# facebookresearch/jepa

Measured on AMD Instinct MI355X. Metric: V-JEPA pretrain clips/sec (fwd+bwd+EMA), higher is better.
Workload: dtype bf16; 1 GPU; V-JEPA pretrain step ViT-L/16 16x224x224, B=24/GPU, 2 multiblock masks (vitl16.yaml); global_batch=24, per_gpu_batch=24, parallelism=dp1, hw_queues=4

## Files before the change

### jepa_amd/csrc/attention.hip

```cpp
#include "attn_common.hpp"

template <int HDP, int NBUF, int RS>
__global__ __launch_bounds__(256) void attn_fwd_sm_kernel(const bf16_t* __restrict__ qkv_all,
                                                          bf16_t* __restrict__ o_all, float* __restrict__ lse2_all,
                                                          AttnSegs sg, int H, int hd, float sc) {
  constexpr int QT = 2, NT = 256;
  using RT = RowTile<HDP, NT>;
  constexpr int DIST = NBUF - 1;
  static_assert(RT::CAN_FULL, "tile items must be a multiple of the workgroup size");
  constexpr bool PSUM = RS == 1;
  constexpr int NDMA = RT::NIT, BUFB = 2 * RT::BYTES;
  __shared__ __attribute__((aligned(16))) char smem[NBUF * BUFB];
  const TrFrag<HDP> trf(threadIdx.x & 63);
  constexpr int KS = HDP / 32, DT = HeadTiles<HDP>::DT;
  const int tid = threadIdx.x, lane = tid & 63, w = tid >> 6;
  const int li = lane & 15, g = lane >> 4;
  const AttnWg wg = attn_wg(sg, H);
  const int S = wg.S, qb = wg.blk;
  const int64_t rs = (int64_t)3 * H * hd, os = (int64_t)H * hd;
  const bf16_t* qbase = wg.rows(qkv_all, rs, hd);
  const bf16_t* kbase = qbase + os;
  const int q0 = qb * 128 + w * (16 * QT);

  bf16x8_t qf[QT][KS];
#pragma unroll
  for (int qt = 0; qt < QT; qt++)
#pragma unroll
    for (int ks = 0; ks < KS; ks++) {
      const int q = q0 + qt * 16 + li, d0 = ks * 32 + 8 * g;
      qf[qt][ks] = scale_frag(load_frag_global(qbase + (int64_t)q * rs + d0, q < S && d0 < hd), sc);
    }

  f32x4_t oacc[QT][DT];
#pragma unroll
  for (int qt = 0; qt < QT; qt++)
#pragma unroll
    for (int dt = 0; dt < DT; dt++) oacc[qt][dt] = (f32x4_t){0.f, 0.f, 0.f, 0.f};
  float mrun[QT], lrun[QT];
  f32x4_t lacc[QT];
  f32x4_t seed[QT];
#pragma unroll
  for (int qt = 0; qt < QT; qt++) {
    mrun[qt] = 0.f;
    lrun[qt] = 0.f;
    lacc[qt] = (f32x4_t){0.f, 0.f, 0.f, 0.f};
    seed[qt] = (f32x4_t){0.f, 0.f, 0.f, 0.f};
  }

  const int nt = (S + 63) / 64;
  const TileDma<HDP, NT, PSUM> dma(tid, hd);
  if constexpr (PSUM) dma.template fill_ypad<NBUF>(smem, tid);
  auto issue = [&](const int tile, const int buf_off, auto full_tag) {
    const bf16_t* kt = kbase + (int64_t)tile * 64 * rs;
    dma.template issue<decltype(full_tag)::value>(kt, rs, kt + os, rs, 0, S - tile * 64, smem + buf_off);
  };
  __builtin_amdgcn_s_waitcnt(0x0f70);
#pragma unroll
  for (int d = 0; d < DIST; d++)
    if (d < nt) issue(d, d * BUFB, std::false_type{});
  RingCursor<NBUF, BUFB> ring;
  const bool wave_live = qb * 128 + dma.wu * (16 * QT) < S;

  auto iter = [&](const int t, auto fast_tag, auto first_tag) {
    constexpr bool FAST = decltype(fast_tag)::value, FIRST = decltype(first_tag)::value;
    const int k0 = t * 64;
    char* k_lds = smem + ring.cur;
    char* v_lds = k_lds + RT::BYTES;
    if (DIST >= 2 && (FAST || t + 1 < nt)) wait_vmcnt<2 * NDMA>();
    else wait_vmcnt<0>();
    lgkm_barrier();
    if constexpr (FAST) issue(t + DIST, ring.nxt, std::true_type{});
    else if (t + DIST < nt) issue(t + DIST, ring.nxt, std::false_type{});
    ring.advance();
    if (!wave_live) return;
    f32x4_t sacc[QT][4];
#pragma unroll
    for (int kt = 0; kt < 4; kt++)
#pragma unroll
      for (int ks = 0; ks < KS; ks++) {
        const bf16x8_t kf = RT::frag(k_lds, kt * 16 + li, ks * 4 + g);
#pragma unroll
        for (int qt = 0; qt < QT; qt++)
          sacc[qt][kt] = __builtin_amdgcn_mfma_f32_16x16x32_bf16(kf, qf[qt][ks], ks == 0 ? seed[qt] : sacc[qt][kt], 0, 0, 0);
      }
    if constexpr (!FAST) {
      if (k0 + 64 > S) {
#pragma unroll
        for (int qt = 0; qt < QT; qt++)
#pragma unroll
          for (int kt = 0; kt < 4; kt++)
#pragma unroll
            for (int r = 0; r < 4; r++)
              if (k0 + kt * 16 + 4 * g + r >= S) sacc[qt][kt][r] = -INFINITY;
      }
    }
    u32x4_t pw[QT][2];
    f32x2_t ls2[QT];
    auto exps = [&](const int qt) __attribute__((always_inline)) {
      ls2[qt] = (f32x2_t){0.f, 0.f};
#pragma unroll
      for (int c = 0; c < 2; c++)
#pragma unroll
        for (int k2 = 0; k2 < 2; k2++)
#pragma unroll
          for (int hf = 0; hf < 2; hf++) {
            const int kt = 2 * c + k2;
            const f32x2_t e = {__builtin_amdgcn_exp2f(sacc[qt][kt][2 * hf]), __builtin_amdgcn_exp2f(sacc[qt][kt][2 * hf + 1])};
            if constexpr (RS == 0) ls2[qt] += e;
            pw[qt][c][2 * k2 + hf] = cvt_pk_bf16(e[0], e[1]);
          }
    };
    bool rebase = FIRST;
    if constexpr (!FIRST) {
      uint32_t orw = 0;
#pragma unroll
      for (int qt = 0; qt < QT; qt++) {
        exps(qt);
        orw |= (pw[qt][0][0] | pw[qt][0][1] | pw[qt][0][2]) | (pw[qt][0][3] | pw[qt][1][0] | pw[qt][1][1]) |
               (pw[qt][1][2] | pw[qt][1][3]);
      }
      rebase = __any((orw & 0x40004000u) != 0);
    }
    if (rebase) {
#pragma unroll
      for (int qt = 0; qt < QT; qt++) {
        float mx = -INFINITY;
#pragma unroll
        for (int kt = 0; kt < 4; kt++)
#pragma unroll
          for (int r = 0; r < 4; r++) mx = fmaxf(mx, sacc[qt][kt][r]);
        mx = fmaxf(mx, __shfl_xor(mx, 16, 64));
        mx = fmaxf(mx, __shfl_xor(mx, 32, 64));
        float shift = mx + SM_HEADROOM;
        if constexpr (!FIRST) {
          shift = fmaxf(shift, 0.f);
          const float alpha = __builtin_amdgcn_exp2f(-shift);
          lrun[qt] *= alpha;
          if constexpr (RS == 2) lacc[qt] *= alpha;
#pragma unroll
          for (int dt = 0; dt < DT; dt++) oacc[qt][dt] *= alpha;
        }
        mrun[qt] += shift;
        seed[qt] = (f32x4_t){-mrun[qt], -mrun[qt], -mrun[qt], -mrun[qt]};
#pragma unroll
        for (int kt = 0; kt < 4; kt++) sacc[qt][kt] -= (f32x4_t){shift, shift, shift, shift};
        exps(qt);
      }
    }
    bf16x8_t pf[QT][2];
#pragma unroll
    for (int qt = 0; qt < QT; qt++) {
      if constexpr (RS == 0) lrun[qt] += ls2[qt][0] + ls2[qt][1];
      pf[qt][0] = __builtin_bit_cast(bf16x8_t, pw[qt][0]);
      pf[qt][1] = __builtin_bit_cast(bf16x8_t, pw[qt][1]);
    }
#pragma unroll
    for (int c = 0; c < 2; c++)
#pragma unroll
      for (int dt = 0; dt < DT; dt++) {
        const bf16x8_t vf = trf.load(v_lds, c * 32, dt * 16);
#pragma unroll
        for (int qt = 0; qt < QT; qt++)
          oacc[qt][dt] = __builtin_amdgcn_mfma_f32_16x16x32_bf16(vf, pf[qt][c], oacc[qt][dt], 0, 0, 0);
      }
    if constexpr (RS == 2) {
      const u32x4_t one4 = {0x3F803F80u, 0x3F803F80u, 0x3F803F80u, 0x3F803F80u};
      const bf16x8_t ones = __builtin_bit_cast(bf16x8_t, one4);
#pragma unroll
      for (int c = 0; c < 2; c++)
#pragma unroll
        for (int qt = 0; qt < QT; qt++) lacc[qt] = __builtin_amdgcn_mfma_f32_16x16x32_bf16(ones, pf[qt][c], lacc[qt], 0, 0, 0);
    }
  };
  const int nfull = S / 64;
  const int t_fast = nfull - DIST > 0 ? nfull - DIST : 0;
  int t = 1;
  if (t_fast > 0) iter(0, std::true_type{}, std::true_type{});
  else iter(0, std::false_type{}, std::true_type{});
  for (; t < t_fast; t++) iter(t, std::true_type{}, std::false_type{});
  for (; t < nt; t++) iter(t, std::false_type{}, std::false_type{});

#pragma unroll
  for (int qt = 0; qt < QT; qt++) {
    float l;
    if constexpr (PSUM) {
      l = __shfl(oacc[qt][1][0], 32 + li, 64);
    } else if constexpr (RS == 2) {
      l = lacc[qt][0];
    } else {
      l = lrun[qt];
      l += __shfl_xor(l, 16, 64);
      l += __shfl_xor(l, 32, 64);
    }
    const int q = q0 + qt * 16 + li;
    if (q < S) {
      store_acc_row<DT>(wg.rows(o_all, os, hd) + q * os, oacc[qt], g, hd, 1.0f / l);
      if (g == 0 && lse2_all) wg.stats(lse2_all, H)[q] = mrun[qt] + log2f(l);
    }
  }
}

template <int HDP, int KT>
__global__ __launch_bounds__(256) void attn_bwd_dkdv_kernel(const bf16_t* __restrict__ qkv_all,
                                                            const bf16_t* __restrict__ dout_all,
                                                            const float* __restrict__ lse2_all,
                                                            const float* __restrict__ delta_all,
                                                            bf16_t* __restrict__ dqkv_all, AttnSegs sg, int H, int hd,
                                                            float sc, float scale, float* __restrict__ colkv) {
  constexpr int BUFB = 2 * RowTile<HDP>::BYTES;
  __shared__ __attribute__((aligned(16))) char smem[2 * BUFB + 2 * 2 * 64 * 4];
  float* stat = (float*)(smem + 2 * BUFB);
  const TrFrag<HDP> trf(threadIdx.x & 63);
  constexpr int KS = HDP / 32, DT = HeadTiles<HDP>::DT;
  const int tid = threadIdx.x, lane = tid & 63, w = tid >> 6;
  const int li = lane & 15, g = lane >> 4;
  const AttnWg wg = attn_wg(sg, H);
  const int S = wg.S, kb = wg.blk;
  const int64_t rs = (int64_t)3 * H * hd, os = (int64_t)H * hd;
  const bf16_t* qbase = wg.rows(qkv_all, rs, hd);
  const bf16_t* kbase = qbase + os;
  const bf16_t* vbase = kbase + os;
  const bf16_t* dobase = wg.rows(dout_all, os, hd);
  const float* lse_b = wg.stats(lse2_all, H);
  const float* dl_b = wg.stats(delta_all, H);
  int key[KT];
  bool key_ok[KT];
#pragma unroll
  for (int kt = 0; kt < KT; kt++) {
    key[kt] = kb * (64 * KT) + (w * KT + kt) * 16 + li;
    key_ok[kt] = key[kt] < S;
  }

  bf16x8_t kf[KT][KS], vf[KT][KS];
#pragma unroll
  for (int kt = 0; kt < KT; kt++)
#pragma unroll
    for (int ks = 0; ks < KS; ks++) {
      const int d0 = ks * 32 + 8 * g;
      kf[kt][ks] = load_frag_global(kbase + (int64_t)key[kt] * rs + d0, key_ok[kt] && d0 < hd);
      vf[kt][ks] = load_frag_global(vbase + (int64_t)key[kt] * rs + d0, key_ok[kt] && d0 < hd);
      kf[kt][ks] = scale_frag(kf[kt][ks], sc);
    }
  f32x4_t dvacc[KT][DT], dkacc[KT][DT];
#pragma unroll
  for (int kt = 0; kt < KT; kt++)
#pragma unroll
    for (int dt = 0; dt < DT; dt++) {
      dvacc[kt][dt] = (f32x4_t){0.f, 0.f, 0.f, 0.f};
      dkacc[kt][dt] = (f32x4_t){0.f, 0.f, 0.f, 0.f};
    }

  float lse_r = 0.f, dl_r = 0.f;
  const int nt = (S + 63) / 64;
  const bool wave_live = kb * (64 * KT) + __builtin_amdgcn_readfirstlane(w) * (16 * KT) < S;
  const TileDma<HDP, 256> dma(tid, hd);
  auto load_stats = [&](int r0) {
    if (tid < 64) {
      const int q = r0 + tid;
      lse_r = q < S ? lse_b[q] : INFINITY;
      dl_r = q < S ? -dl_b[q] : 0.f;
    }
  };
  __builtin_amdgcn_s_waitcnt(0x0f70);
  load_stats(0);
  dma.template issue<false>(qbase, rs, dobase, os, 0, S, smem);
  if (tid < 64) {
    stat[tid] = lse_r;
    stat[64 + tid] = dl_r;
  }
  if (nt > 1) load_stats(64);

  for (int t = 0; t < nt; t++) {
    char* q_lds = smem + (t & 1) * BUFB;
    char* do_lds = q_lds + RowTile<HDP>::BYTES;
    const float* lse_s = stat + (t & 1) * 128;
    const float* dl_s = lse_s + 64;
    wait_vmcnt<0>();
    lgkm_barrier();
    if (t + 1 < nt) {
      if (tid < 64) {
        stat[((t + 1) & 1) * 128 + tid] = lse_r;
        stat[((t + 1) & 1) * 128 + 64 + tid] = dl_r;
      }
      if (t + 2 < nt) load_stats((t + 2) * 64);
      if ((t + 1) * 64 + 64 <= S) dma.template issue<true>(qbase, rs, dobase, os, (t + 1) * 64, S, smem + ((t + 1) & 1) * BUFB);
      else dma.template issue<false>(qbase, rs, dobase, os, (t + 1) * 64, S, smem + ((t + 1) & 1) * BUFB);
    }

    if (!wave_live) continue;
#pragma unroll
    for (int c = 0; c < 2; c++) {
      if (c == 1 && t * 64 + 32 >= S) break;
      float pv[KT][2][4], dsv[KT][2][4];
#pragma unroll
      for (int q2 = 0; q2 < 2; q2++) {
        const int qt = 2 * c + q2;
        const float4 lse4 = *(const float4*)(lse_s + qt * 16 + 4 * g);
        const float4 ndl4 = *(const float4*)(dl_s + qt * 16 + 4 * g);
        f32x4_t sacc[KT], dpacc[KT];
#pragma unroll
        for (int kt = 0; kt < KT; kt++) {
          sacc[kt] = (f32x4_t){-lse4.x, -lse4.y, -lse4.z, -lse4.w};
          dpacc[kt] = (f32x4_t){ndl4.x, ndl4.y, ndl4.z, ndl4.w};
        }
#pragma unroll
        for (int ks = 0; ks < KS; ks++) {
          const bf16x8_t qa = RowTile<HDP>::frag(q_lds, qt * 16 + li, ks * 4 + g);
          const bf16x8_t da = RowTile<HDP>::frag(do_lds, qt * 16 + li, ks * 4 + g);
#pragma unroll
          for (int kt = 0; kt < KT; kt++) {
            sacc[kt] = __builtin_amdgcn_mfma_f32_16x16x32_bf16(qa, kf[kt][ks], sacc[kt], 0, 0, 0);
            dpacc[kt] = __builtin_amdgcn_mfma_f32_16x16x32_bf16(da, vf[kt][ks], dpacc[kt], 0, 0, 0);
          }
        }
#pragma unroll
        for (int kt = 0; kt < KT; kt++)
#pragma unroll
          for (int hf = 0; hf < 2; hf++) {
            const f32x2_t dpv = {dpacc[kt][2 * hf], dpacc[kt][2 * hf + 1]};
            const f32x2_t e = {__builtin_amdgcn_exp2f(sacc[kt][2 * hf]), __builtin_amdgcn_exp2f(sacc[kt][2 * hf + 1])};
            const f32x2_t ds = e * dpv;
            pv[kt][q2][2 * hf] = e[0];
            pv[kt][q2][2 * hf + 1] = e[1];
            dsv[kt][q2][2 * hf] = ds[0];
            dsv[kt][q2][2 * hf + 1] = ds[1];
          }
      }
      bf16x8_t pfr[KT], dfr[KT];
#pragma unroll
      for (int kt = 0; kt < KT; kt++) {
        pfr[kt] = pack_frag(pv[kt][0], pv[kt][1]);
        dfr[kt] = pack_frag(dsv[kt][0], dsv[kt][1]);
      }
#pragma unroll
      for (int dt = 0; dt < DT; dt++) {
        const bf16x8_t dot_f = trf.load(do_lds, c * 32, dt * 16);
        const bf16x8_t qt_f = trf.load(q_lds, c * 32, dt * 16);
#pragma unroll
        for (int kt = 0; kt < KT; kt++) {
          dvacc[kt][dt] = __builtin_amdgcn_mfma_f32_16x16x32_bf16(dot_f, pfr[kt], dvacc[kt][dt], 0, 0, 0);
          dkacc[kt][dt] = __builtin_amdgcn_mfma_f32_16x16x32_bf16(qt_f, dfr[kt], dkacc[kt][dt], 0, 0, 0);
        }
      }
    }
  }

  if (colkv != nullptr) {
    float ck[DT][4], cv[DT][4];
#pragma unroll
    for (int dt = 0; dt < DT; dt++)
#pragma unroll
      for (int r = 0; r < 4; r++) {
        float a = 0.f, c = 0.f;
#pragma unroll
        for (int kt = 0; kt < KT; kt++) {
          a += key_ok[kt] ? dkacc[kt][dt][r] : 0.f;
          c += key_ok[kt] ? dvacc[kt][dt][r] : 0.f;
        }
        ck[dt][r] = row16_sum(a);
        cv[dt][r] = row16_sum(c);
      }
    lgkm_barrier();
    float* red = (float*)smem;
    if (li == 0) {
#pragma unroll
      for (int dt = 0; dt < DT; dt++)
#pragma unroll
        for (int r = 0; r < 4; r++) {
          red[(w * 2 + 0) * HDP + dt * 16 + 4 * g + r] = ck[dt][r];
          red[(w * 2 + 1) * HDP + dt * 16 + 4 * g + r] = cv[dt][r];
        }
    }
    lgkm_barrier();
    if (tid < 2 * HDP) {
      const int which = tid / HDP, d = tid % HDP;
      if (d < hd) {
        float t = red[(0 * 2 + which) * HDP + d] + red[(1 * 2 + which) * HDP + d] + red[(2 * 2 + which) * HDP + d] +
                  red[(3 * 2 + which) * HDP + d];
        if (which == 0) t *= scale;
        wg.colrow(colkv, 2 * os, hd)[(int64_t)which * os + d] = t;
      }
    }
  }
#pragma unroll
  for (int kt = 0; kt < KT; kt++) {
    if (key_ok[kt]) {
      bf16_t* dkp = wg.rows(dqkv_all, rs, hd) + key[kt] * rs + os;
      bf16_t* dvp = dkp + os;
#pragma unroll
      for (int dt = 0; dt < DT; dt++) {
        const int d = dt * 16 + 4 * g;
        if (d < hd) {
          u32x2_t a, c;
          a[0] = cvt_pk_bf16(dkacc[kt][dt][0] * scale, dkacc[kt][dt][1] * scale);
          a[1] = cvt_pk_bf16(dkacc[kt][dt][2] * scale, dkacc[kt][dt][3] * scale);
          c[0] = cvt_pk_bf16(dvacc[kt][dt][0], dvacc[kt][dt][1]);
          c[1] = cvt_pk_bf16(dvacc[kt][dt][2], dvacc[kt][dt][3]);
          *(u32x2_t*)(dkp + d) = a;
          *(u32x2_t*)(dvp + d) = c;
        }
      }
    }
  }
}

template <int HDP>
__global__ __launch_bounds__(256) void attn_bwd_dq_kernel(const bf16_t* __restrict__ qkv_all,
                                                          const bf16_t* __restrict__ o_all,
                                                          const bf16_t* __restrict__ dout_all,
                                                          const float* __restrict__ lse2_all,
                                                          float* __restrict__ delta_all,
                                                          bf16_t* __restrict__ dqkv_all, AttnSegs sg, int H, int hd,
                                                          float sc, float scale, float* __restrict__ colq) {
  constexpr int NBUF = HDP <= 64 ? 3 : 2, DIST = NBUF - 1, BUFB = 2 * RowTile<HDP>::BYTES;
  __shared__ __attribute__((aligned(16))) char smem[NBUF * BUFB];
  const TrFrag<HDP> trf(threadIdx.x & 63);
  constexpr int KS = HDP / 32, DT = HeadTiles<HDP>::DT;
  constexpr int QW = 2;
  const int tid = threadIdx.x, lane = tid & 63, w = tid >> 6;
  const int li = lane & 15, g = lane >> 4;
  const AttnWg wg = attn_wg(sg, H);
  const int S = wg.S, qb = wg.blk;
  const int64_t rs = (int64_t)3 * H * hd, os = (int64_t)H * hd;
  const bf16_t* qbase = wg.rows(qkv_all, rs, hd);
  const bf16_t* kbase = qbase + os;
  const bf16_t* vbase = kbase + os;
  const bf16_t* dobase = wg.rows(dout_all, os, hd);
  const bf16_t* obase = wg.rows(o_all, os, hd);
  const float* lse_b = wg.stats(lse2_all, H);
  float* dl_b = wg.stats(delta_all, H);
  const int q0 = qb * (64 * QW) + w * (16 * QW);

  bf16x8_t qf[QW][KS], dof[QW][KS];
  float lse_q[QW], dl_q[QW];
#pragma unroll
  for (int qt = 0; qt < QW; qt++) {
    const int q = q0 + qt * 16 + li;
    float dsum = 0.f;
#pragma unroll
    for (int ks = 0; ks < KS; ks++) {
      const int d0 = ks * 32 + 8 * g;
      const bool ok = q < S && d0 < hd;
      qf[qt][ks] = load_frag_global(qbase + (int64_t)q * rs + d0, ok);
      dof[qt][ks] = load_frag_global(dobase + (int64_t)q * os + d0, ok);
      const u32x4_t ov = __builtin_bit_cast(u32x4_t, load_frag_global(obase + (int64_t)q * os + d0, ok));
      const u32x4_t dv = __builtin_bit_cast(u32x4_t, dof[qt][ks]);
#pragma unroll
      for (int j = 0; j < 4; j++) dsum += bf_lo(ov[j]) * bf_lo(dv[j]) + bf_hi(ov[j]) * bf_hi(dv[j]);
    }
    dsum += __shfl_xor(dsum, 16, 64);
    dsum += __shfl_xor(dsum, 32, 64);
    lse_q[qt] = q < S ? lse_b[q] : INFINITY;
    dl_q[qt] = q < S ? dsum : 0.f;
    if (g == 0 && q < S) dl_b[q] = dsum;
#pragma unroll
    for (int ks = 0; ks < KS; ks++) qf[qt][ks] = scale_frag(qf[qt][ks], sc);
  }
  f32x4_t dqacc[QW][DT];
#pragma unroll
  for (int qt = 0; qt < QW; qt++)
#pragma unroll
    for (int dt = 0; dt < DT; dt++) dqacc[qt][dt] = (f32x4_t){0.f, 0.f, 0.f, 0.f};

  f32x4_t ndl4[QW];
  f32x4_t nls4[QW];
#pragma unroll
  for (int qt = 0; qt < QW; qt++) {
    ndl4[qt] = (f32x4_t){-dl_q[qt], -dl_q[qt], -dl_q[qt], -dl_q[qt]};
    nls4[qt] = (f32x4_t){-lse_q[qt], -lse_q[qt], -lse_q[qt], -lse_q[qt]};
  }
  const int nt = (S + 63) / 64;
  const bool wave_live = qb * (64 * QW) + __builtin_amdgcn_readfirstlane(w) * (16 * QW) < S;
  const TileDma<HDP, 256> dma(tid, hd);
  constexpr int NDMA2 = 2 * TileDma<HDP, 256>::NDMA;
  __builtin_amdgcn_s_waitcnt(0x0f70);
#pragma unroll
  for (int d = 0; d < DIST; d++)
    if (d < nt) dma.template issue<false>(kbase, rs, vbase, rs, d * 64, S, smem + d * BUFB);
  RingCursor<NBUF, BUFB> ring;

  for (int t = 0; t < nt; t++) {
    const int k0 = t * 64;
    char* k_lds = smem + ring.cur;
    char* v_lds = k_lds + RowTile<HDP>::BYTES;
    if (DIST >= 2 && t + 1 < nt) wait_vmcnt<NDMA2>();
    else wait_vmcnt<0>();
    lgkm_barrier();
    if (t + DIST < nt) {
      if ((t + DIST) * 64 + 64 <= S) dma.template issue<true>(kbase, rs, vbase, rs, (t + DIST) * 64, S, smem + ring.nxt);
      else dma.template issue<false>(kbase, rs, vbase, rs, (t + DIST) * 64, S, smem + ring.nxt);
    }
    ring.advance();
    if (!wave_live) continue;
#pragma unroll
    for (int c = 0; c < 2; c++) {
      if (c == 1 && k0 + 32 >= S) break;
      f32x4_t sacc[QW][2], dpacc[QW][2];
#pragma unroll
      for (int qt = 0; qt < QW; qt++)
#pragma unroll
        for (int k2 = 0; k2 < 2; k2++) {
          sacc[qt][k2] = nls4[qt];
          dpacc[qt][k2] = ndl4[qt];
        }
#pragma unroll
      for (int k2 = 0; k2 < 2; k2++)
#pragma unroll
        for (int ks = 0; ks < KS; ks++) {
          const int kt = 2 * c + k2;
          const bf16x8_t ka = RowTile<HDP>::frag(k_lds, kt * 16 + li, ks * 4 + g);
          const bf16x8_t va = RowTile<HDP>::frag(v_lds, kt * 16 + li, ks * 4 + g);
#pragma unroll
          for (int qt = 0; qt < QW; qt++) {
            sacc[qt][k2] = __builtin_amdgcn_mfma_f32_16x16x32_bf16(ka, qf[qt][ks], sacc[qt][k2], 0, 0, 0);
            dpacc[qt][k2] = __builtin_amdgcn_mfma_f32_16x16x32_bf16(va, dof[qt][ks], dpacc[qt][k2], 0, 0, 0);
          }
        }
#pragma unroll
      for (int qt = 0; qt < QW; qt++) {
#pragma unroll
        for (int k2 = 0; k2 < 2; k2++)
#pragma unroll
          for (int hf = 0; hf < 2; hf++) {
            const f32x2_t sv = {sacc[qt][k2][2 * hf], sacc[qt][k2][2 * hf + 1]};
            const f32x2_t dpv = {dpacc[qt][k2][2 * hf], dpacc[qt][k2][2 * hf + 1]};
            const f32x2_t e = {__builtin_amdgcn_exp2f(sv[0]), __builtin_amdgcn_exp2f(sv[1])};
            const f32x2_t ds = e * dpv;
            sacc[qt][k2][2 * hf] = ds[0];
            sacc[qt][k2][2 * hf + 1] = ds[1];
          }
      }
      if (k0 + 64 > S) {
        asm volatile("" ::: "memory");
#pragma unroll
        for (int qt = 0; qt < QW; qt++)
#pragma unroll
          for (int k2 = 0; k2 < 2; k2++)
#pragma unroll
            for (int r = 0; r < 4; r++)
              if (k0 + (2 * c + k2) * 16 + 4 * g + r >= S) sacc[qt][k2][r] = 0.f;
      }
      bf16x8_t dsf[QW];
#pragma unroll
      for (int qt = 0; qt < QW; qt++) dsf[qt] = pack_frag(sacc[qt][0], sacc[qt][1]);
#pragma unroll
      for (int dt = 0; dt < DT; dt++) {
        const bf16x8_t ktf = trf.load(k_lds, c * 32, dt * 16);
#pragma unroll
        for (int qt = 0; qt < QW; qt++)
          dqacc[qt][dt] = __builtin_amdgcn_mfma_f32_16x16x32_bf16(ktf, dsf[qt], dqacc[qt][dt], 0, 0, 0);
      }
    }
  }

  if (colq != nullptr) {
    float cq[DT][4];
#pragma unroll
    for (int dt = 0; dt < DT; dt++)
#pragma unroll
      for (int r = 0; r < 4; r++) {
        cq[dt][r] = row16_sum(dqacc[0][dt][r] + dqacc[1][dt][r]);
      }
    lgkm_barrier();
    float* red = (float*)smem;
    if (li == 0) {
#pragma unroll
      for (int dt = 0; dt < DT; dt++)
#pragma unroll
        for (int r = 0; r < 4; r++) red[w * HDP + dt * 16 + 4 * g + r] = cq[dt][r];
    }
    lgkm_barrier();
    if (tid < hd) wg.colrow(colq, os, hd)[tid] =
        (red[tid] + red[HDP + tid] + red[2 * HDP + tid] + red[3 * HDP + tid]) * scale;
  }
#pragma unroll
  for (int qt = 0; qt < QW; qt++) {
    const int q = q0 + qt * 16 + li;
    if (q < S) store_acc_row<DT>(wg.rows(dqkv_all, rs, hd) + q * rs, dqacc[qt], g, hd, scale);
  }
}

static int pick_hdp(int64_t hd) { return hd <= 32 ? 32 : (hd <= 64 ? 64 : (hd <= 80 ? 96 : (hd <= 128 ? 128 : 0))); }
constexpr float LOG2E = 1.4426950408889634f;
static int attn_check_hd(const char* who, int64_t hd) {
  VJ_CHECK_ARG(hd % 8 == 0 && pick_hdp(hd) != 0, "%s: head_dim=%ld unsupported (need %%8==0, <=128)", who, (long)hd);
  return 0;
}

template <int HDP_, int NBUF_, int RS_, int KT_>
struct AttnClass { static constexpr int HDP = HDP_, NBUF = NBUF_, RS = RS_, KT = KT_; };
template <class F>
static inline int with_head_dim(int64_t hd, F&& f) {
  switch (pick_hdp(hd)) {
    case 32: return hd == 24 ? f(AttnClass<32, 3, 1, 2>{}) : f(AttnClass<32, 3, 2, 2>{});
    case 64: return f(AttnClass<64, 2, 2, 1>{});
    case 96: return f(AttnClass<96, 2, 2, 1>{});
    default: return f(AttnClass<128, 2, 2, 1>{});
  }
}
static int dkdv_kt(int64_t hd) { return with_head_dim(hd, [](auto c) { return decltype(c)::KT; }); }
static int64_t attn_rows_end(const vj_seg_t* segs, int64_t n_segs) {
  int64_t rows_end = 0;
  for (int64_t i = 0; i < n_segs; i++)
    if (segs[i].B * segs[i].S > 0 && segs[i].row0 + segs[i].B * segs[i].S > rows_end) rows_end = segs[i].row0 + segs[i].B * segs[i].S;
  return rows_end;
}

static int make_segs(const vj_seg_t* segs, int64_t n_segs, int64_t H, int64_t rows_per_block, AttnSegs* out, int64_t* nblk,
                     const char* who) {
  VJ_CHECK_ARG(segs != nullptr && n_segs >= 1 && n_segs <= VJ_ATTN_MAX_SEGS, "%s: 1..%d segments", who, VJ_ATTN_MAX_SEGS);
  int k = 0;
  int64_t tot = 0, col = 0;
  for (int64_t i = 0; i < n_segs; i++) {
    VJ_CHECK_ARG(segs[i].B >= 0 && segs[i].S >= 0 && segs[i].row0 >= 0, "%s: bad segment %ld", who, (long)i);
    if (segs[i].B * segs[i].S == 0) continue;
    const int64_t nb = cdiv64(segs[i].S, rows_per_block);
    tot += segs[i].B * H * nb;
    VJ_CHECK_ARG(tot < (1ll << 31) && segs[i].S < (1ll << 31), "%s: grid too large", who);
    out->blk_end[k] = (int)tot;
    out->S[k] = (int)segs[i].S;
    out->nb[k] = (int)nb;
    out->row0[k] = segs[i].row0;
    out->col0[k] = col;
    col += segs[i].B * nb;
    k++;
  }
  for (int i = k; i < VJ_ATTN_MAX_SEGS; i++) {
    out->blk_end[i] = (int)tot;
    out->S[i] = 0;
    out->nb[i] = 1;
    out->row0[i] = 0;
    out->col0[i] = 0;
  }
  out->n = k;
  *nblk = tot;
  return 0;
}

extern "C" int vj_attn_fwd_segs(const void* qkv, void* o, float* lse2, const vj_seg_t* segs, int64_t n_segs, int64_t H,
                                int64_t hd, float scale, hipStream_t stream) {
  if (int rc = attn_check_hd("vj_attn_fwd", hd)) return rc;
  VJ_CHECK_ARG(H > 0, "vj_attn_fwd: bad dims");
  AttnSegs sg;
  int64_t nblk = 0;
  if (int rc = make_segs(segs, n_segs, H, 128, &sg, &nblk, "vj_attn_fwd")) return rc;
  if (nblk == 0) return 0;
  const float sc = scale < 0.f ? 1.0f : scale * LOG2E;
  with_head_dim(hd, [&](auto c) {
    using C = decltype(c);
    hipLaunchKernelGGL((attn_fwd_sm_kernel<C::HDP, C::NBUF, C::RS>), dim3((unsigned)nblk), dim3(256), 0, stream, (const bf16_t*)qkv,
                       (bf16_t*)o, lse2, sg, (int)H, (int)hd, sc);
    return 0;
  });
  VJ_LAUNCH_CHECK("vj_attn_fwd");
  return 0;
}

extern "C" int vj_attn_fwd(const void* qkv, void* o, float* lse2, int64_t B, int64_t S, int64_t H, int64_t hd,
                           float scale, hipStream_t stream) {
  VJ_CHECK_ARG(B >= 0 && S >= 0 && H > 0, "vj_attn_fwd: bad dims");
  const vj_seg_t one = {0, B, S};
  return vj_attn_fwd_segs(qkv, o, lse2, &one, 1, H, hd, scale, stream);
}

extern "C" int64_t vj_attn_bwd_segs_ws_bytes(const vj_seg_t* segs, int64_t n_segs, int64_t H, int64_t hd) {
  (void)hd;
  if (segs == nullptr || n_segs <= 0) return 0;
  return attn_rows_end(segs, n_segs) * H * 4;
}
extern "C" int64_t vj_attn_bwd_ws_bytes(int64_t B, int64_t S, int64_t H) {
  const vj_seg_t one = {0, B, S};
  return vj_attn_bwd_segs_ws_bytes(&one, 1, H, 0);
}

extern "C" int vj_attn_bwd_colsum_rows(int64_t B, int64_t S, int64_t hd, int64_t* rows_q, int64_t* rows_kv) {
  VJ_CHECK_ARG(rows_q != nullptr && rows_kv != nullptr, "vj_attn_bwd_colsum_rows: bad arguments");
  if (int rc = attn_check_hd("vj_attn_bwd_colsum_rows", hd)) return rc;
  *rows_q = B * cdiv64(S, 128);
  *rows_kv = B * cdiv64(S, 64 * dkdv_kt(hd));
  return 0;
}

extern "C" int vj_attn_bwd_segs(const void* qkv, const void* o, const void* dout, const float* lse2, void* dqkv,
                                const vj_seg_t* segs, int64_t n_segs, int64_t H, int64_t hd, float scale, void* ws,
                                int64_t ws_bytes, float* colq, float* colkv, hipStream_t stream) {
  if (int rc = attn_check_hd("vj_attn_bwd", hd)) return rc;
  VJ_CHECK_ARG(H > 0 && (colq == nullptr) == (colkv == nullptr), "vj_attn_bwd: bad arguments");
  const int kt = dkdv_kt(hd);
  AttnSegs sq, sk;
  int64_t gq = 0, gk = 0;
  if (int rc = make_segs(segs, n_segs, H, 128, &sq, &gq, "vj_attn_bwd")) return rc;
  if (int rc = make_segs(segs, n_segs, H, 64 * kt, &sk, &gk, "vj_attn_bwd")) return rc;
  if (gq == 0) return 0;
  VJ_CHECK_ARG(ws != nullptr && ws_bytes >= attn_rows_end(segs, n_segs) * H * 4, "vj_attn_bwd: workspace too small");
  float* delta = (float*)ws;
  const bool pre = scale < 0.f;
  const float sabs = fabsf(scale);
  const float sc = pre ? 1.0f : sabs * LOG2E;
  const float kscale = pre ? 1.0f / LOG2E : sabs;
  with_head_dim(hd, [&](auto c) {
    using C = decltype(c);
    hipLaunchKernelGGL((attn_bwd_dq_kernel<C::HDP>), dim3((unsigned)gq), dim3(256), 0, stream, (const bf16_t*)qkv, (const bf16_t*)o,
                       (const bf16_t*)dout, lse2, delta, (bf16_t*)dqkv, sq, (int)H, (int)hd, sc, sabs, colq);
    hipLaunchKernelGGL((attn_bwd_dkdv_kernel<C::HDP, C::KT>), dim3((unsigned)gk), dim3(256), 0, stream, (const bf16_t*)qkv,
                       (const bf16_t*)dout, lse2, delta, (bf16_t*)dqkv, sk, (int)H, (int)hd, sc, kscale, colkv);
    return 0;
  });
  VJ_LAUNCH_CHECK("vj_attn_bwd");
  return 0;
}

extern "C" int vj_attn_bwd(const void* qkv, const void* o, const void* dout, const float* lse2, void* dqkv,
                           int64_t B, int64_t S, int64_t H, int64_t hd, float scale, void* ws, int64_t ws_bytes,
                           hipStream_t stream) {
  VJ_CHECK_ARG(B >= 0 && S >= 0, "vj_attn_bwd: bad dims");
  const vj_seg_t one = {0, B, S};
  return vj_attn_bwd_segs(qkv, o, dout, lse2, dqkv, &one, 1, H, hd, scale, ws, ws_bytes, nullptr, nullptr, stream);
}

extern "C" int vj_attn_bwd_colsum(const void* qkv, const void* o, const void* dout, const float* lse2, void* dqkv,
                                  int64_t B, int64_t S, int64_t H, int64_t hd, float scale, void* ws, int64_t ws_bytes,
                                  float* colq, float* colkv, hipStream_t stream) {
  VJ_CHECK_ARG(colq != nullptr && colkv != nullptr && B >= 0 && S >= 0, "vj_attn_bwd_colsum: bad arguments");
  const vj_seg_t one = {0, B, S};
  return vj_attn_bwd_segs(qkv, o, dout, lse2, dqkv, &one, 1, H, hd, scale, ws, ws_bytes, colq, colkv, stream);
}
```

### jepa_amd/csrc/lds_pipe.hpp

```cpp
#pragma once
#include "common.hpp"

#define LDS_PART_BYTES 16384

__device__ __forceinline__ void cfence() { asm volatile("" ::: "memory"); }

__device__ __forceinline__ void section_barrier() {
  cfence();
  __builtin_amdgcn_sched_barrier(0);
  __builtin_amdgcn_s_barrier();
  __builtin_amdgcn_sched_barrier(0);
  cfence();
}
__device__ __forceinline__ void lgkm_barrier() {
  cfence();
  __builtin_amdgcn_s_waitcnt(0xc07f);
  __builtin_amdgcn_s_barrier();
  cfence();
}

template <int N>
__device__ __forceinline__ void wait_vmcnt() {
  asm volatile("s_waitcnt vmcnt(%0)" ::"n"(N) : "memory");
}

__device__ __forceinline__ unsigned lds_addr(const char* p) {
  return (unsigned)(size_t)(__attribute__((address_space(3))) const char*)p;
}

__device__ __forceinline__ void dma16_v(const void* gsrc, unsigned lds_base) {
  asm volatile("s_mov_b32 m0, %0\n\ts_nop 0\n\tglobal_load_lds_dwordx4 %1, off" ::"s"(lds_base), "v"(gsrc) : "memory");
}
__device__ __forceinline__ void dma16_sv(const void* sbase, unsigned voff, unsigned lds_base) {
  asm volatile("s_mov_b32 m0, %0\n\ts_nop 0\n\tglobal_load_lds_dwordx4 %1, %2" ::"s"(lds_base), "v"(voff), "s"(sbase) : "memory");
}
```

Before: 335.4 clips/s.

## Stream attention bwd stats via LDS DMA ring and hoist tile prefetch

The dK/dV backward kernel now loads the per-query LSE and negated delta statistics with direct global-to-LDS dword DMA, issued by two waves and kept in a ring buffer parameterized by NBUF. This replaces the register staging path and its extra LDS stores. The dQ kernel stores the negated delta so dK/dV can use it without negating. The dQ kernel also issues its K/V tile prefetch before loading Q/dO/O fragments and splits the delta computation into a second loop, so global loads overlap. All head dims use NBKV=2 for now, which keeps a distance of one. That makes the change mainly a restructuring of stat loading plus earlier prefetch rather than a deeper pipeline.

```diff
diff --git a/jepa_amd/csrc/attention.hip b/jepa_amd/csrc/attention.hip
--- a/jepa_amd/csrc/attention.hip
+++ b/jepa_amd/csrc/attention.hip
@@ -200,16 +200,16 @@
   }
 }
 
-template <int HDP, int KT>
+template <int HDP, int KT, int NBUF>
 __global__ __launch_bounds__(256) void attn_bwd_dkdv_kernel(const bf16_t* __restrict__ qkv_all,
                                                             const bf16_t* __restrict__ dout_all,
                                                             const float* __restrict__ lse2_all,
-                                                            const float* __restrict__ delta_all,
+                                                            const float* __restrict__ ndelta_all,
                                                             bf16_t* __restrict__ dqkv_all, AttnSegs sg, int H, int hd,
                                                             float sc, float scale, float* __restrict__ colkv) {
-  constexpr int BUFB = 2 * RowTile<HDP>::BYTES;
-  __shared__ __attribute__((aligned(16))) char smem[2 * BUFB + 2 * 2 * 64 * 4];
-  float* stat = (float*)(smem + 2 * BUFB);
+  constexpr int DIST = NBUF - 1, BUFB = 2 * RowTile<HDP>::BYTES, STATB = 2 * 64 * 4;
+  __shared__ __attribute__((aligned(16))) char smem[NBUF * BUFB + NBUF * STATB];
+  char* stat = smem + NBUF * BUFB;
   const TrFrag<HDP> trf(threadIdx.x & 63);
   constexpr int KS = HDP / 32, DT = HeadTiles<HDP>::DT;
   const int tid = threadIdx.x, lane = tid & 63, w = tid >> 6;
@@ -222,7 +222,7 @@
   const bf16_t* vbase = kbase + os;
   const bf16_t* dobase = wg.rows(dout_all, os, hd);
   const float* lse_b = wg.stats(lse2_all, H);
-  const float* dl_b = wg.stats(delta_all, H);
+  const float* dl_b = wg.stats(ndelta_all, H);
   int key[KT];
   bool key_ok[KT];
 #pragma unroll
@@ -230,6 +230,24 @@
     key[kt] = kb * (64 * KT) + (w * KT + kt) * 16 + li;
     key_ok[kt] = key[kt] < S;
   }
+
+  const int nt = (S + 63) / 64;
+  const TileDma<HDP, 256> dma(tid, hd);
+  constexpr int NDMA2 = 2 * TileDma<HDP, 256>::NDMA;
+  const bool stat_wave = dma.wu < 2;
+  const float* stat_src = dma.wu == 0 ? lse_b : dl_b;
+  auto issue = [&](const int tile, const int img_off, const int stat_off, auto full_tag) {
+    constexpr bool FULL = decltype(full_tag)::value;
+    if (stat_wave) {
+      char* row = stat + stat_off + dma.wu * 256;
+      if (FULL || tile * 64 + lane < S) dma4_sv(stat_src + tile * 64, (unsigned)lane * 4u, lds_addr(row));
+      else ((float*)row)[lane] = dma.wu == 0 ? INFINITY : 0.f;
+    }
+    dma.template issue<FULL>(qbase, rs, dobase, os, tile * 64, S, smem + img_off);
+  };
+#pragma unroll
+  for (int d = 0; d < DIST; d++)
+    if (d < nt) issue(d, d * BUFB, d * STATB, std::false_type{});
 
   bf16x8_t kf[KT][KS], vf[KT][KS];
 #pragma unroll
@@ -250,42 +268,29 @@
       dkacc[kt][dt] = (f32x4_t){0.f, 0.f, 0.f, 0.f};
     }
 
-  float lse_r = 0.f, dl_r = 0.f;
-  const int nt = (S + 63) / 64;
   const bool wave_live = kb * (64 * KT) + __builtin_amdgcn_readfirstlane(w) * (16 * KT) < S;
-  const TileDma<HDP, 256> dma(tid, hd);
-  auto load_stats = [&](int r0) {
-    if (tid < 64) {
-      const int q = r0 + tid;
-      lse_r = q < S ? lse_b[q] : INFINITY;
-      dl_r = q < S ? -dl_b[q] : 0.f;
-    }
-  };
   __builtin_amdgcn_s_waitcnt(0x0f70);
-  load_stats(0);
-  dma.template issue<false>(qbase, rs, dobase, os, 0, S, smem);
-  if (tid < 64) {
-    stat[tid] = lse_r;
-    stat[64 + tid] = dl_r;
-  }
-  if (nt > 1) load_stats(64);
+  RingCursor<NBUF, BUFB> ring;
+  RingCursor<NBUF, STATB> sring;
 
   for (int t = 0; t < nt; t++) {
-    char* q_lds = smem + (t & 1) * BUFB;
+    char* q_lds = smem + ring.cur;
     char* do_lds = q_lds + RowTile<HDP>::BYTES;
-    const float* lse_s = stat + (t & 1) * 128;
+    const float* lse_s = (const float*)(stat + sring.cur);
     const float* dl_s = lse_s + 64;
-    wait_vmcnt<0>();
+    if (DIST >= 2 && t + DIST - 1 < nt) {
+      if (stat_wave) wait_vmcnt<(DIST - 1) * (NDMA2 + 1)>();
+      else wait_vmcnt<(DIST - 1) * NDMA2>();
+    } else {
+      wait_vmcnt<0>();
+    }
     lgkm_barrier();
-    if (t + 1 < nt) {
-      if (tid < 64) {
-        stat[((t + 1) & 1) * 128 + tid] = lse_r;
-        stat[((t + 1) & 1) * 128 + 64 + tid] = dl_r;
-      }
-      if (t + 2 < nt) load_stats((t + 2) * 64);
-      if ((t + 1) * 64 + 64 <= S) dma.template issue<true>(qbase, rs, dobase, os, (t + 1) * 64, S, smem + ((t + 1) & 1) * BUFB);
-      else dma.template issue<false>(qbase, rs, dobase, os, (t + 1) * 64, S, smem + ((t + 1) & 1) * BUFB);
-    }
+    if (t + DIST < nt) {
+      if ((t + DIST) * 64 + 64 <= S) issue(t + DIST, ring.nxt, sring.nxt, std::true_type{});
+      else issue(t + DIST, ring.nxt, sring.nxt, std::false_type{});
+    }
+    ring.advance();
+    sring.advance();
 
     if (!wave_live) continue;
 #pragma unroll
@@ -431,28 +436,44 @@
   float* dl_b = wg.stats(delta_all, H);
   const int q0 = qb * (64 * QW) + w * (16 * QW);
 
+  const int nt = (S + 63) / 64;
+  const TileDma<HDP, 256> dma(tid, hd);
+  constexpr int NDMA2 = 2 * TileDma<HDP, 256>::NDMA;
+#pragma unroll
+  for (int d = 0; d < DIST; d++)
+    if (d < nt) dma.template issue<false>(kbase, rs, vbase, rs, d * 64, S, smem + d * BUFB);
+
   bf16x8_t qf[QW][KS], dof[QW][KS];
+  u32x4_t of[QW][KS];
   float lse_q[QW], dl_q[QW];
 #pragma unroll
   for (int qt = 0; qt < QW; qt++) {
     const int q = q0 + qt * 16 + li;
-    float dsum = 0.f;
 #pragma unroll
     for (int ks = 0; ks < KS; ks++) {
       const int d0 = ks * 32 + 8 * g;
       const bool ok = q < S && d0 < hd;
       qf[qt][ks] = load_frag_global(qbase + (int64_t)q * rs + d0, ok);
       dof[qt][ks] = load_frag_global(dobase + (int64_t)q * os + d0, ok);
-      const u32x4_t ov = __builtin_bit_cast(u32x4_t, load_frag_global(obase + (int64_t)q * os + d0, ok));
+      of[qt][ks] = __builtin_bit_cast(u32x4_t, load_frag_global(obase + (int64_t)q * os + d0, ok));
+    }
+    lse_q[qt] = q < S ? lse_b[q] : INFINITY;
+  }
+#pragma unroll
+  for (int qt = 0; qt < QW; qt++) {
+    const int q = q0 + qt * 16 + li;
+    float dsum = 0.f;
+#pragma unroll
+    for (int ks = 0; ks < KS; ks++) {
+      const u32x4_t ov = of[qt][ks];
       const u32x4_t dv = __builtin_bit_cast(u32x4_t, dof[qt][ks]);
 #pragma unroll
       for (int j = 0; j < 4; j++) dsum += bf_lo(ov[j]) * bf_lo(dv[j]) + bf_hi(ov[j]) * bf_hi(dv[j]);
     }
     dsum += __shfl_xor(dsum, 16, 64);
     dsum += __shfl_xor(dsum, 32, 64);
-    lse_q[qt] = q < S ? lse_b[q] : INFINITY;
     dl_q[qt] = q < S ? dsum : 0.f;
-    if (g == 0 && q < S) dl_b[q] = dsum;
+    if (g == 0 && q < S) dl_b[q] = -dsum;
 #pragma unroll
     for (int ks = 0; ks < KS; ks++) qf[qt][ks] = scale_frag(qf[qt][ks], sc);
   }
@@ -469,14 +490,8 @@
     ndl4[qt] = (f32x4_t){-dl_q[qt], -dl_q[qt], -dl_q[qt], -dl_q[qt]};
     nls4[qt] = (f32x4_t){-lse_q[qt], -lse_q[qt], -lse_q[qt], -lse_q[qt]};
   }
-  const int nt = (S + 63) / 64;
   const bool wave_live = qb * (64 * QW) + __builtin_amdgcn_readfirstlane(w) * (16 * QW) < S;
-  const TileDma<HDP, 256> dma(tid, hd);
-  constexpr int NDMA2 = 2 * TileDma<HDP, 256>::NDMA;
   __builtin_amdgcn_s_waitcnt(0x0f70);
-#pragma unroll
-  for (int d = 0; d < DIST; d++)
-    if (d < nt) dma.template issue<false>(kbase, rs, vbase, rs, d * 64, S, smem + d * BUFB);
   RingCursor<NBUF, BUFB> ring;
 
   for (int t = 0; t < nt; t++) {
@@ -587,15 +602,15 @@
   return 0;
 }
 
-template <int HDP_, int NBUF_, int RS_, int KT_>
-struct AttnClass { static constexpr int HDP = HDP_, NBUF = NBUF_, RS = RS_, KT = KT_; };
+template <int HDP_, int NBUF_, int RS_, int KT_, int NBKV_>
+struct AttnClass { static constexpr int HDP = HDP_, NBUF = NBUF_, RS = RS_, KT = KT_, NBKV = NBKV_; };
 template <class F>
 static inline int with_head_dim(int64_t hd, F&& f) {
   switch (pick_hdp(hd)) {
-    case 32: return hd == 24 ? f(AttnClass<32, 3, 1, 2>{}) : f(AttnClass<32, 3, 2, 2>{});
-    case 64: return f(AttnClass<64, 2, 2, 1>{});
-    case 96: return f(AttnClass<96, 2, 2, 1>{});
-    default: return f(AttnClass<128, 2, 2, 1>{});
+    case 32: return hd == 24 ? f(AttnClass<32, 3, 1, 2, 2>{}) : f(AttnClass<32, 3, 2, 2, 2>{});
+    case 64: return f(AttnClass<64, 2, 2, 1, 2>{});
+    case 96: return f(AttnClass<96, 2, 2, 1, 2>{});
+    default: return f(AttnClass<128, 2, 2, 1, 2>{});
   }
 }
 static int dkdv_kt(int64_t hd) { return with_head_dim(hd, [](auto c) { return decltype(c)::KT; }); }
@@ -702,7 +717,7 @@
     using C = decltype(c);
     hipLaunchKernelGGL((attn_bwd_dq_kernel<C::HDP>), dim3((unsigned)gq), dim3(256), 0, stream, (const bf16_t*)qkv, (const bf16_t*)o,
                        (const bf16_t*)dout, lse2, delta, (bf16_t*)dqkv, sq, (int)H, (int)hd, sc, sabs, colq);
-    hipLaunchKernelGGL((attn_bwd_dkdv_kernel<C::HDP, C::KT>), dim3((unsigned)gk), dim3(256), 0, stream, (const bf16_t*)qkv,
+    hipLaunchKernelGGL((attn_bwd_dkdv_kernel<C::HDP, C::KT, C::NBKV>), dim3((unsigned)gk), dim3(256), 0, stream, (const bf16_t*)qkv,
                        (const bf16_t*)dout, lse2, delta, (bf16_t*)dqkv, sk, (int)H, (int)hd, sc, kscale, colkv);
     return 0;
   });
diff --git a/jepa_amd/csrc/lds_pipe.hpp b/jepa_amd/csrc/lds_pipe.hpp
--- a/jepa_amd/csrc/lds_pipe.hpp
+++ b/jepa_amd/csrc/lds_pipe.hpp
@@ -34,3 +34,6 @@
 __device__ __forceinline__ void dma16_sv(const void* sbase, unsigned voff, unsigned lds_base) {
   asm volatile("s_mov_b32 m0, %0\n\ts_nop 0\n\tglobal_load_lds_dwordx4 %1, %2" ::"s"(lds_base), "v"(voff), "s"(sbase) : "memory");
 }
+__device__ __forceinline__ void dma4_sv(const void* sbase, unsigned voff, unsigned lds_base) {
+  asm volatile("s_mov_b32 m0, %0\n\ts_nop 0\n\tglobal_load_lds_dword %1, %2" ::"s"(lds_base), "v"(voff), "s"(sbase) : "memory");
+}
```

Result: no change. 336.1 clips/s, median of 3 (+0.2%).
